# heli-sudoo/HKD-MPC

Hardware: AMD Instinct MI355X
Metric: batched DDP iters/sec (fwd+bwd), 4-phase 200-knot HKD fp64, batch=4096 (higher is better)
Workload: dtype f64

## Files before the change

### hkd-mpc_amd/csrc/hsddp_sweep.hip

```cpp
#include "hsddp_wave.h"

namespace hsddp {

using namespace hkd;

namespace sweep {

#ifndef HSDDP_STAMPS
#define HSDDP_STAMPS 0
#endif
#ifndef SWEEP_WPB2_WPE
#define SWEEP_WPB2_WPE 1
#endif
#if HSDDP_STAMPS
#define STAMP(n)                                                                              \
    do {                                                                                      \
        __builtin_amdgcn_sched_barrier(0);                                                    \
        unsigned long long t_;                                                                \
        asm volatile("s_waitcnt lgkmcnt(0)\n\ts_memtime %0\n\ts_waitcnt lgkmcnt(0)" : "=s"(t_)::"memory"); \
        __builtin_amdgcn_sched_barrier(0);                                                    \
        if (threadIdx.x == 0) {                                                               \
            if ((n) > 0) S.st[n] += t_ - S.tprev;                                             \
            S.tprev = t_;                                                                     \
        }                                                                                     \
    } while (0)
#else
#define STAMP(n) \
    do {         \
    } while (0)
#endif

#define SSYNC()                              \
    do {                                     \
        asm volatile("" ::: "memory");       \
        __builtin_amdgcn_sched_barrier(0);   \
    } while (0)

#define CSYNC()                                              \
    do {                                                     \
        asm volatile("s_waitcnt lgkmcnt(0)" ::: "memory");   \
        __builtin_amdgcn_s_barrier();                        \
        asm volatile("" ::: "memory");                       \
        __builtin_amdgcn_sched_barrier(0);                   \
    } while (0)

constexpr int HC = 12;
constexpr int MS = 26;
constexpr int TS = 14;
constexpr int WS = 25;
constexpr int V_SE = LQ_SE, V_D = 104, V_LX = 128, V_LU = 152, V_RB = 176, VW = 200;
static_assert(LQ_BW + 36 == V_D && LQ_LX + 24 == V_LX && LQ_LU + 24 == V_LU && LQ_RB + 24 == V_RB, "image layout");

template <typename real>
struct alignas(16) Lds {
    real img[2][VW];
    real zero[32];
    struct alignas(16) Item {
        real TI[24 * TS];
        real MI[25 * MS];
        real du[24];
        real pc[8];
    } it[2];
#if HSDDP_STAMPS
    unsigned long long st[12], tprev;
#endif
};
static_assert(sizeof(Lds<double>) <= 20480, "two waves per SIMD on 160 KB of LDS need <= 20 KB per wave");

template <typename real>
struct alignas(16) LdsCS {
    real img[2][2][VW];
    real zero[32];
    struct alignas(16) Item {
        real TI[24 * TS];
        real MZ[2][25 * MS];
        real du[24];
        real pc[8];
    } it[2];
    int fl[2];
};
static_assert(sizeof(LdsCS<double>) <= 40960, "four split workgroups per CU on 160 KB of LDS need <= 40 KB each");

template <typename real>
struct Pieces {
    static constexpr int E = 16 / sizeof(real);
    static constexpr int NA = V_D / E, ND = NX / E, NR = (LQW - V_D) / E, NP = NA + ND + NR;
    static constexpr int NI = (2 * NP + 63) / 64;
    static_assert(NP * E == VW && V_D % E == 0, "16-byte pieces");
};

template <typename real> struct Prec;
template <> struct Prec<double> {
    static DEV const double *lq(const Bufs &d) { return d.lq; }
    static DEV double *K(const Bufs &d) { return d.K; }
    static DEV const double *def(const Bufs &d, int b) { return kdbuf(work_buf(d, b)); }
    static constexpr int LQS = LQW;
};
template <> struct Prec<float> {
    static DEV const float *lq(const Bufs &d) { return d.lq32; }
    static DEV float *K(const Bufs &d) { return d.K32; }
    static DEV const float *def(const Bufs &d, int) { return d.def32; }
    static constexpr int LQS = LQW32;
};

template <typename real>
struct Item {
    int b;
    bool act;
    real reg;
    real *K;
    double *dU;
};

template <typename real>
struct Phase {
    int cmask;
    int xmask;
    real lxd;
    real xw;
    real dtr;
    real dtrz;
};


template <typename real, typename ItemT>
DEV void load_phase(const Params &p, const Bufs &d, ItemT &I, int b, int i, int pp, Phase<real> &ph)
{
    const int *cs = d.contacts + ((size_t)b * (p.P + 1) + i) * 4;
    int c[4];
#pragma unroll
    for (int l = 0; l < 4; ++l) c[l] = cs[l];
    ph.cmask = 0;
#pragma unroll
    for (int l = 0; l < 4; ++l) ph.cmask |= (c[l] != 0) << l;
    SSYNC();
    if (pp < 8) {
        const int cl = (ph.cmask >> (pp & 3)) & 1;
        I.pc[pp] = pp < 4 ? (cl ? (real)p.dt_m : (real)0) : (cl ? (real)0 : (real)p.dt);
    }
    SSYNC();
    const int pos = pp & 15, cq = (ph.cmask >> ((pos / 3) & 3)) & 1;
    ph.dtr = (real)(p.dt * (cq ? p.r_grf : p.r_qJd));
    const int cz = (ph.cmask >> ((pp < HC ? pp : 0) / 3)) & 1;
    ph.dtrz = (real)(p.dt * (cz ? p.r_qJd : p.r_grf));
    const int r = pp < NX ? pp : 0;
    double dg = p.dt * (r < 12 ? kparams()->qbase[r] : p.q_qJ * (1 - ((ph.cmask >> ((r - 12) / 3)) & 1)));
    ph.xmask = 0;
    ph.xw = 0;
    if (r >= 3 && r < 6) {
        const double fw = p.dt * (p.foot_gain * kparams()->foot_w[r - 3]);
#pragma unroll
        for (int l = 0; l < 4; ++l) dg += c[l] ? fw : 0.0;
        ph.xmask = ph.cmask;
        ph.xw = (real)fw;
    } else if (r >= 12) {
        const int m = r - 12;
        const double w = ((ph.cmask >> (m / 3)) & 1) ? p.dt * (p.foot_gain * kparams()->foot_w[m % 3]) : 0.0;
        dg += w;
        ph.xmask = 1;
        ph.xw = (real)w;
    }
    ph.lxd = (real)dg;
}

template <typename real>
DEV void fetch(Lds<real> &S, const real *rec0, const real *def0, const real *rec1, const real *def1, int lane)
{
    using PC = Pieces<real>;
    asm volatile("s_waitcnt lgkmcnt(0)" ::: "memory");
#pragma unroll
    for (int t = 0; t < PC::NI; ++t) {
        const int n = 64 * t + lane;
        if (n < 2 * PC::NP) {
            const int e = n >= PC::NP, q = n - e * PC::NP;
            const real *rec = e ? rec1 : rec0, *def = e ? def1 : def0;
            const real *src = q < PC::NA ? rec + PC::E * q : q < PC::NA + PC::ND ? def + PC::E * (q - PC::NA)
                                                                                 : rec + PC::E * (q - PC::ND);
            lds_dma16(src, (unsigned)(size_t)(&S.img[0][0]) + 1024u * t);
        }
    }
}

template <int W, typename real>
DEV void fetch_cs(LdsCS<real> &S, int q, const real *rec0, const real *def0, const real *rec1, const real *def1,
                  int lane)
{
    using PC = Pieces<real>;
    constexpr int H = (PC::NI + 1) / 2;
#pragma unroll
    for (int u = 0; u < H; ++u) {
        const int t = W * H + u;
        const int n = 64 * t + lane;
        if (t < PC::NI && n < 2 * PC::NP) {
            const int e = n >= PC::NP, qq = n - e * PC::NP;
            const real *rec = e ? rec1 : rec0, *def = e ? def1 : def0;
            const real *src = qq < PC::NA ? rec + PC::E * qq : qq < PC::NA + PC::ND ? def + PC::E * (qq - PC::NA)
                                                                                    : rec + PC::E * (qq - PC::ND);
            lds_dma16(src, (unsigned)(size_t)(&S.img[q][0][0]) + 1024u * t);
        }
    }
}

DEV constexpr int rb_index(int a, int b)
{
    return (a < b ? a : b) == 0 ? (a > b ? a : b) : (a < b ? a : b) == 1 ? 2 + (a > b ? a : b) : 5;
}

struct Lane {
    int lane, e, pp, pos;
    bool row;
    bool qlane;
    int rb[3];
    int xc0, xkind;
};

constexpr unsigned CS_COLS1 = (1u << 0) | (1u << 3) | (1u << 4) | (1u << 5) | (1u << 8) | (1u << 9) | (1u << 10) |
                              (1u << 11) | (1u << 18) | (1u << 19) | (1u << 21) | (1u << 22);
DEV constexpr int cs_wave(int c) { return (int)((CS_COLS1 >> c) & 1u); }
template <int W>
DEV constexpr bool cs_mine(int c) { return W < 0 || cs_wave(c) == W; }

template <int W = -1, typename real>
DEV void emit_SA(real (&acc)[NX], const real (&x)[NX], const real (&cf)[8], real dt)
{
    auto sw_row = [&](auto I) {
        constexpr int i = I;
        static_for<17>([&](auto Q) {
            if constexpr (cs_mine<W>(sw_col(Q))) vfma<sw_at(i, Q)>(acc[sw_col(Q)], cf, x[6 + i]);
        });
    };
    auto se_row = [&](auto I) {
        constexpr int i = I;
        static_for<5>([&](auto Q) {
            if constexpr (cs_mine<W>(se_col(Q))) vfma<V_SE + 5 * i + Q>(acc[se_col(Q)], cf, x[i]);
        });
    };
    sw_row(std::integral_constant<int, 0>{});
    se_row(std::integral_constant<int, 0>{});
    sw_row(std::integral_constant<int, 1>{});
    se_row(std::integral_constant<int, 1>{});
    sw_row(std::integral_constant<int, 2>{});
    se_row(std::integral_constant<int, 2>{});
    static_for<3>([&](auto A) {
        if constexpr (cs_mine<W>(9 + A)) acc[9 + A] = __builtin_fma(x[3 + A], dt, acc[9 + A]);
    });
}

template <int Q0 = 0, int Q1 = HC, typename real>
DEV void emit_Bc(real (&acc)[HC], real y6, real y7, real y8, const real *y9, const real *y12, const real (&bv)[4],
                 const real (&bq)[4], const real (&cf)[8])
{
#pragma unroll
    for (int q = Q0; q < Q1; ++q) acc[q] = __builtin_fma(y12[q], bq[q / 3], acc[q]);
#pragma unroll
    for (int q = Q0; q < Q1; ++q) acc[q] = __builtin_fma(y9[q % 3], bv[q / 3], acc[q]);
    static_for<Q1 - Q0>([&](auto Q) { vfma<bw_at(0, Q0 + Q)>(acc[Q0 + Q], cf, y6); });
    static_for<Q1 - Q0>([&](auto Q) { vfma<bw_at(1, Q0 + Q)>(acc[Q0 + Q], cf, y7); });
    static_for<Q1 - Q0>([&](auto Q) { vfma<bw_at(2, Q0 + Q)>(acc[Q0 + Q], cf, y8); });
}

template <typename real>
DEV void eliminate(real (&w)[HC], real (&w2)[HC], unsigned long long &bad)
{
    constexpr bool F64 = sizeof(real) == 8;
    constexpr int CH = F64 ? 13 : 9;
    real r, e, nf, nf2;
    {
        const real piv = row_bcast<0>(w[0]);
        bad |= __builtin_amdgcn_ballot_w64(!(piv > (real)1e-9));
        asm_rcp(r, piv);
        asm_nfma1(e, piv, r);
        asm_newton(r, e);
        if constexpr (F64) {
            asm_nfma1(e, piv, r);
            asm_newton(r, e);
        }
        asm_nmul(nf, w[0], r);
        asm_nmul(nf2, w2[0], r);
    }
    static_for<HC>([&](auto J) {
        constexpr int j = J, jn = j + 1;
        constexpr bool nx = jn < HC;
        real pivn = 0, rn = 0, en = 0, nfn = 0, nf2n = 0;
        if constexpr (nx) {
            bfma<j>(w2[jn], w[jn], nf2);
            fmac_row_bcast<j, false>(w[jn], nf);
        }
        constexpr int NO = nx ? HC - 2 - j : 0;
        constexpr int NT = (2 * NO > CH + 1) ? 2 * NO : CH + 1;
        static_for<NT>([&](auto T) {
            constexpr int t = T, i = jn + 1 + t / 2;
            if constexpr (t < 2 * NO) {
                if constexpr (t % 2 == 0)
                    bfma<j>(w2[i], w[i], nf2);
                else
                    fmac_row_bcast<j, false>(w[i], nf);
            }
            if constexpr (nx) {
                if constexpr (t == 1) pivn = row_bcast<(nx ? jn : 0)>(w[jn]);
                if constexpr (t == 3) asm_rcp(rn, pivn);
                if constexpr (t == 5) asm_nfma1(en, pivn, rn);
                if constexpr (t == 7) asm_newton(rn, en);
                if constexpr (F64 && t == 9) asm_nfma1(en, pivn, rn);
                if constexpr (F64 && t == 11) asm_newton(rn, en);
                if constexpr (t == CH) {
                    asm_nmul(nfn, w[jn], rn);
                    asm_nmul(nf2n, w2[jn], rn);
                }
            }
        });
        w[j] = nf;
        w2[j] = nf2;
        if constexpr (nx) {
            bad |= __builtin_amdgcn_ballot_w64(!(pivn > (real)1e-9));
            nf = nfn;
            nf2 = nf2n;
        }
    });
    static_for<HC - 1>([&](auto Jr) {
        constexpr int j = HC - 1 - Jr;
        static_for<j>([&](auto Ii) {
            constexpr int i = j - 1 - Ii;
            bfma<j>(w2[i], w[i], w2[j]);
        });
    });
}

template <int W, bool DV, typename real, typename LdsT>
DEV void knot(const Params &p, LdsT &S, const Lane &L, const Phase<real> &ph, const Item<real> &it, int kc,
              real (&h)[NX], real &g, bool &live, bool first, bool more, int ib, int par, const real *nrec0,
              const real *ndef0, const real *nrec1, const real *ndef1, double &dvs)
{
    constexpr bool CS = W >= 0;
    constexpr int Q0 = CS ? 6 * W : 0, Q1 = CS ? Q0 + 6 : HC;
    auto &I = S.it[L.e];
    const real *img;
    real *ma = nullptr, *za = nullptr;
    if constexpr (CS) {
        img = S.img[ib][L.e];
        ma = I.MZ[par];
        za = I.MZ[par ^ 1];
    } else {
        img = S.img[L.e];
    }
    auto MA = [&]() -> real * { if constexpr (CS) return ma; else return I.MI; };
    auto ZA = [&]() -> real * { if constexpr (CS) return za; else return I.MI; };
    const int pp = L.pp, pos = L.pos;
    const real dt = (real)p.dt;
    const real reg = it.reg;
    if constexpr (!CS) STAMP(0);
    if (first) {
        asm volatile("s_waitcnt vmcnt(0)" ::: "memory");
        if constexpr (CS) CSYNC();
    }
    real cf[8];
#pragma unroll
    for (int k = 0; k < 8; ++k) cf[k] = img[16 * k + pos];
    real bv[4], bq[4];
#pragma unroll
    for (int l = 0; l < 4; ++l) { bv[l] = I.pc[l]; bq[l] = I.pc[4 + l]; }
    if constexpr (!CS) STAMP(1);
    real t[HC], ga[4] = {g, 0, 0, 0};
#pragma unroll
    for (int q = 0; q < HC; ++q) t[q] = 0;
    emit_Bc<Q0, Q1>(t, h[6], h[7], h[8], h + 9, h + 12, bv, bq, cf);
    static_for<NX>([&](auto C) { vfma<V_D + C>(ga[C & 3], cf, h[C]); });
    const real gn = (ga[0] + ga[1]) + (ga[2] + ga[3]);
    pin(t);
    real h9[NX];
#pragma unroll
    for (int j = 0; j < 9; ++j) h9[j] = h[j];
#pragma unroll
    for (int j = 9; j < NX; ++j) h9[j] = 0;
    SSYNC();
    real (&m)[NX] = h;
    emit_SA<W>(m, h9, cf, dt);
    pin(t);
    pin(m);
    if (L.row) {
        static_for<NX>([&](auto C) {
            if constexpr (cs_mine<W>(C)) MA()[pp * MS + C] = m[C];
        });
        if constexpr (W <= 0) MA()[pp * MS + NX] = gn;
#pragma unroll
        for (int q = Q0; q < Q1; ++q) I.TI[pp * TS + q] = t[q];
    }
    if constexpr (CS) CSYNC(); else SSYNC();
    if constexpr (!CS) STAMP(2);
    const int pc = pp < MS - 1 ? pp : MS - 1;
    real mc[NX];
#pragma unroll
    for (int j = 0; j < NX; ++j) mc[j] = MA()[j * MS + pc];
    real w2[HC];
#pragma unroll
    for (int l = 0; l < 4; ++l) {
        const real *lcp = pp == NX ? img + V_LU + (((ph.cmask >> l) & 1) ? 3 * l : 12 + 3 * l) : S.zero;
#pragma unroll
        for (int a = 0; a < 3; ++a) w2[3 * l + a] = lcp[a];
    }
    emit_SA<W>(m, mc, cf, dt);
    emit_Bc(w2, mc[6], mc[7], mc[8], mc + 9, mc + 12, bv, bq, cf);
    pin(m);
    pin(w2);
    if constexpr (!CS) STAMP(3);
    if (pp <= NX) {
#pragma unroll
        for (int c = 0; c < NX; ++c)
            if (cs_mine<W>(c)) ZA()[pp * MS + c] = m[c];
        if constexpr (W <= 0) {
            ZA()[pp * MS + NX] = 0;
            ZA()[pp * MS + NX + 1] = 0;
        }
    }
    SSYNC();
    if (L.row) {
        real *zr = ZA() + pp * MS;
        if (cs_mine<W>(pp)) lds_add(zr + pp, ph.lxd + reg);
#pragma unroll
        for (int t2 = 0; t2 < 4; ++t2) {
            const int xc = L.xkind == 1 ? L.xc0 + 3 * t2 : L.xc0;
            if (((ph.xmask >> t2) & 1) && cs_mine<W>(xc)) lds_add(zr + xc, -ph.xw);
        }
    }
    if constexpr (CS) CSYNC(); else SSYNC();
    const real *zrow = L.row ? ZA() + pp * MS : S.zero;
    real qxx[NX], zc[NX];
    if constexpr (CS) {
        static_for<NX>([&](auto C) {
            if constexpr (cs_mine<W>(C)) {
                qxx[C] = zrow[C];
                zc[C] = ZA()[C * MS + pc];
            }
        });
        static_for<NX>([&](auto C) {
            if constexpr (cs_mine<W>(C)) qxx[C] = __builtin_fma(zc[C], (real)0.5, qxx[C] * (real)0.5);
        });
    } else {
#pragma unroll
        for (int c = 0; c < NX; ++c) qxx[c] = zrow[c];
#pragma unroll
        for (int c = 0; c < NX; ++c) zc[c] = ZA()[c * MS + pc];
        pin(qxx);
        pin(zc);
#pragma unroll
        for (int c = 0; c < NX; ++c) qxx[c] *= (real)0.5;
#pragma unroll
        for (int c = 0; c < NX; ++c) qxx[c] = __builtin_fma(zc[c], (real)0.5, qxx[c]);
        pin(qxx);
    }
    const real qx = img[V_LX + (L.row ? pp : 0)] + (gn + ZA()[NX * MS + pc]);
    if constexpr (!CS) STAMP(4);
    real tcol[18];
#pragma unroll
    for (int j = 0; j < 18; ++j) tcol[j] = I.TI[(6 + j) * TS + pos];
    real lbr[3];
    const int aq = pos % 3;
#pragma unroll
    for (int a = 0; a < 3; ++a) lbr[a] = (L.qlane ? img + L.rb[a] : S.zero + a)[0] + (a == aq ? ph.dtr + reg : (real)0);
    const int lq = pos / 3;
    real w[HC];
#pragma unroll
    for (int q = 0; q < HC; ++q) w[q] = (L.qlane && lq == q / 3) ? lbr[q % 3] : (real)0;
    emit_Bc(w, tcol[0], tcol[1], tcol[2], tcol + 3, tcol + 6, bv, bq, cf);
    pin(w);
    const bool zl = pp < HC;
    const int du_z = ((ph.cmask >> ((zl ? pp : 0) / 3)) & 1) ? 12 + pp : pp;
    const real quz = img[zl ? V_LU + du_z : V_LU];
    const real qzz = ph.dtrz + reg;
    if (more) {
        if constexpr (CS) fetch_cs<W>(S, ib ^ 1, nrec0, ndef0, nrec1, ndef1, L.lane);
        else fetch(S, nrec0, ndef0, nrec1, ndef1, L.lane);
    }
    if constexpr (!CS) STAMP(5);
    real quxs[HC];
#pragma unroll
    for (int q = 0; q < HC; ++q) quxs[q] = (L.row || (DV && pp == NX)) ? w2[q] : (real)0;
    pin(quxs);
    unsigned long long bad = __builtin_amdgcn_ballot_w64(zl && !(qzz > (real)1e-9));
    eliminate(w, w2, bad);
    const bool okh = L.e ? (bad >> 32) == 0 : (bad & 0xffffffffull) == 0;
    live = live && okh;
    const bool st = live;
    if constexpr (!CS) STAMP(6);
    if (pp == NX)
#pragma unroll
        for (int q = 0; q < HC; ++q) I.du[(((ph.cmask >> (q / 3)) & 1) ? 0 : 12) + q] = w2[q];
    if (zl) I.du[du_z] = -(quz / qzz);
    SSYNC();
    real ka[HC], kb[HC];
#pragma unroll
    for (int q = 0; q < HC; ++q) row_pair_last(w2[q], ka[q], kb[q]);
    real gq4[4] = {qx, 0, 0, 0};
    static_for<HC>([&](auto Q) { bfma<8>(gq4[Q & 3], kb[Q], quxs[Q]); });
    const real gq = (gq4[0] + gq4[1]) + (gq4[2] + gq4[3]);
    if constexpr (DV) {
        real dq = 0;
        static_for<HC>([&](auto Q) { bfma<8>(dq, kb[Q], quxs[Q]); });
        const double v = pp == NX ? (double)dq : zl ? (double)quz * (double)(-(quz / qzz)) : 0.0;
        if (st) dvs += v;
    }
    if constexpr (!CS) STAMP(7);
    if constexpr (CS) {
        static_for<NX>([&](auto C) {
            if constexpr (cs_mine<W>(C)) h[C] = qxx[C];
        });
    } else {
#pragma unroll
        for (int c = 0; c < NX; ++c) h[c] = qxx[c];
    }
    static_for<HC>([&](auto Q) {
        static_for<NX>([&](auto C) {
            constexpr int c = C;
            if constexpr (cs_mine<W>(c)) {
                if constexpr (c < 16)
                    bfma<c & 15>(h[c], ka[Q], quxs[Q]);
                else
                    bfma<c & 15>(h[c], kb[Q], quxs[Q]);
            }
        });
    });
    if constexpr (DV)
        if (!L.row)
            static_for<NX>([&](auto C) {
                if constexpr (cs_mine<W>(C)) h[C] = 0;
            });
    if constexpr (!CS) STAMP(8);
    g = L.row ? gq : (real)0;
    if constexpr (CS)
        if (L.row)
            static_for<NX>([&](auto C) {
                if constexpr (cs_mine<W>(C)) MA()[pp * MS + C] = h[C];
            });
    asm volatile("s_waitcnt vmcnt(0)" ::: "memory");
    if (st) {
        real *Kg = it.K + (size_t)kc * KCW;
        if constexpr (W <= 0) {
#pragma unroll
            for (int q = 0; q < HC; ++q) Kg[q * NX + pos] = ka[q];
        }
        if constexpr (W != 0) {
            if (pos < NX - 16)
#pragma unroll
                for (int q = 0; q < HC; ++q) Kg[q * NX + 16 + pos] = kb[q];
            if (L.row) it.dU[(size_t)kc * NX + pp] = I.du[pp];
        }
    }
    if constexpr (CS) {
        CSYNC();
        static_for<NX>([&](auto C) {
            if constexpr (!cs_mine<W>(C)) h[C] = L.row ? MA()[pp * MS + C] : (real)0;
        });
    }
    SSYNC();
    if constexpr (!CS) STAMP(9);
}

template <typename real, bool EL, bool DV, int CSW = -1, typename LdsT = Lds<real>>
DEV int sweep_pair(const Params &p, const Bufs &d, LdsT &S, const Lane &L, const Item<real> &it, double &dv)
{
    constexpr bool CS = CSW >= 0;
    int ib = 0, par = 0;
    double dvs = 0.0;
    const int pp = L.pp;
    const real *lqg = Prec<real>::lq(d);
    const int b = it.b;
    const int b0 = __builtin_amdgcn_readlane(b, 0), b1 = __builtin_amdgcn_readlane(b, 32);
    const real *defg0 = Prec<real>::def(d, b0), *defg1 = Prec<real>::def(d, b1);
    bool live = it.act;
    int fail = -1;
    real h[NX], g = 0;
    const auto PL = layout_of<EL>(d, b0);
    const int P = PL.P();
    for (int i = P - 1; i >= 0; --i) {
        Phase<real> ph;
        load_phase<real>(p, d, S.it[L.e], b, i, pp, ph);
        const double *rec = d.term + ((size_t)b * p.P + i) * TW;
        if (i == P - 1) {
#pragma unroll
            for (int c = 0; c < NX; ++c) h[c] = L.row ? (real)rec[TM_PHIXX + pp * NX + c] : (real)0;
            g = L.row ? (real)rec[TM_PHIX + pp] : (real)0;
        } else {
            auto &I = S.it[L.e];
            real *WI;
            if constexpr (CS) {
                WI = I.MZ[0];
                CSYNC();
            } else {
                WI = I.MI;
            }
            const double *Px = rec + TM_PX;
            real wr[NX];
#pragma unroll
            for (int c = 0; c < NX; ++c) wr[c] = 0;
            static_for<3>([&](auto Kc) {
                real px[12];
#pragma unroll
                for (int k = 0; k < 12; ++k) px[k] = (real)Px[192 * Kc + 16 * k + L.pos];
                if constexpr (sizeof(real) == 4) dpp_ready(px);
                static_for<8>([&](auto Kk) {
                    static_for<NX>([&](auto Cc) { vfma<NX * Kk + Cc>(wr[Cc], px, h[8 * Kc + Kk]); });
                });
            });
            SSYNC();
            if (L.row) {
#pragma unroll
                for (int c = 0; c < NX; ++c) WI[pp * WS + c] = wr[c];
                WI[pp * WS + NX] = g;
            }
            SSYNC();
            const int pc = pp < NX ? pp : NX;
            real wc[NX];
#pragma unroll
            for (int j = 0; j < NX; ++j) wc[j] = WI[j * WS + pc];
            real vr[NX];
#pragma unroll
            for (int c = 0; c < NX; ++c) vr[c] = 0;
            static_for<3>([&](auto Kc) {
                real px[12];
#pragma unroll
                for (int k = 0; k < 12; ++k) px[k] = (real)Px[192 * Kc + 16 * k + L.pos];
                if constexpr (sizeof(real) == 4) dpp_ready(px);
                static_for<8>([&](auto Jj) {
                    static_for<NX>([&](auto Cc) { vfma<NX * Jj + Cc>(vr[Cc], px, wc[8 * Kc + Jj]); });
                });
            });
            SSYNC();
            if (pp == NX)
#pragma unroll
                for (int c = 0; c < NX; ++c) WI[NX * WS + c] = vr[c];
            SSYNC();
            const real gp = WI[NX * WS + (L.row ? pp : 0)];
#pragma unroll
            for (int c = 0; c < NX; ++c) h[c] = L.row ? (real)rec[TM_PHIXX + pp * NX + c] + vr[c] : (real)0;
            g = L.row ? (real)rec[TM_PHIX + pp] + gp : (real)0;
            SSYNC();
            if constexpr (CS) CSYNC();
        }
        const int N = PL.N(i), s0 = PL.s0(i), k0 = PL.k0(i);
        auto recp = [&](int bb, int k) { return lqg + ((size_t)bb * p.Kc + k0 + k) * Prec<real>::LQS; };
        auto defp0 = [&](int k) { return defg0 + ((size_t)b0 * p.S + s0 + k + 1) * NX; };
        auto defp1 = [&](int k) { return defg1 + ((size_t)b1 * p.S + s0 + k + 1) * NX; };
        if constexpr (CS) fetch_cs<CSW>(S, ib, recp(b0, N - 1), defp0(N - 1), recp(b1, N - 1), defp1(N - 1), L.lane);
        else fetch(S, recp(b0, N - 1), defp0(N - 1), recp(b1, N - 1), defp1(N - 1), L.lane);
        int k = N - 1;
#pragma unroll 1
        for (; k >= 0; --k) {
            const bool more = k > 0;
            const int kn = more ? k - 1 : 0;
            const bool was = live;
            knot<CSW, DV>(p, S, L, ph, it, k0 + k, h, g, live, k == N - 1, more, ib, par, recp(b0, kn), defp0(kn),
                          recp(b1, kn), defp1(kn), dvs);
            if constexpr (CS) {
                ib ^= more ? 1 : 0;
                par ^= 1;
            }
            if (was && !live) fail = k0 + k;
            if (!__builtin_amdgcn_ballot_w64(live)) break;
        }
        asm volatile("s_waitcnt vmcnt(0)" ::: "memory");
        if (!__builtin_amdgcn_ballot_w64(live)) break;
        const real *d0 = (L.e ? defg1 : defg0) + ((size_t)b * p.S + s0) * NX;
        real dc[2] = {d0[L.pos], L.pos < NX - 16 ? d0[16 + L.pos] : (real)0};
        real a = 0;
        static_for<NX>([&](auto Cc) { vfma<Cc>(a, dc, h[Cc]); });
        if (L.row) g += a;
        if (p.store_value && live && L.row && CSW <= 0) {
            double *V = d.value0 + ((size_t)b * p.P + i) * (NX + NN);
#pragma unroll
            for (int c = 0; c < NX; ++c) V[NX + pp * NX + c] = (double)h[c];
            V[pp] = (double)g;
        }
    }
    if constexpr (DV) {
#pragma unroll
        for (int o = 16; o > 0; o >>= 1) dvs += __shfl_xor(dvs, o);
    }
    dv = dvs;
    return it.act ? fail : -1;
}

constexpr int STAGE_SLOTS = 512;

template <typename ItemT>
DEV double *cost_stage(const Params &p, ItemT &item)
{
    const bool fits = p.S <= STAGE_SLOTS && 2 * (size_t)p.S * sizeof(double) <= sizeof(ItemT);
    return fits ? reinterpret_cast<double *>(&item) : nullptr;
}

template <bool EL>
DEV void element_cost(const Params &p, const Bufs &d, int b, int lane, double *stg, double &cost, double &feas)
{
    const auto LY = layout_of<EL>(d, b);
    const int P = LY.P(), g = lane & 31;
    const double *c = d.slot_cost + (size_t)b * p.S, *f = d.slot_feas + (size_t)b * p.S;
    if (stg) {
        const int Sel = LY.S();
#pragma unroll
        for (int t = 0; t < STAGE_SLOTS / 32; ++t) {
            const int sl = g + 32 * t;
            if (sl < Sel) {
                stg[sl] = c[sl];
                stg[p.S + sl] = f[sl];
            }
        }
        __builtin_amdgcn_fence(__ATOMIC_RELEASE, "wavefront");
        __builtin_amdgcn_wave_barrier();
        __builtin_amdgcn_fence(__ATOMIC_ACQUIRE, "wavefront");
        c = stg;
        f = stg + p.S;
    }
    double ci = 0.0, fi = 0.0;
    if (g < P) {
        const int N = LY.N(g), s0 = LY.s0(g);
#pragma unroll 10
        for (int k = 0; k < N; ++k) {
            ci += c[s0 + k];
            fi += f[s0 + k];
        }
        ci += c[s0 + N];
        fi += f[s0 + N];
    }
    cost = 0.0; feas = 0.0;
    for (int i = 0; i < P; ++i) {
        cost += __shfl(ci, (lane & 32) + i);
        feas += __shfl(fi, (lane & 32) + i);
    }
    feas = sqrt(feas);
}

DEV Lane make_lane()
{
    Lane L;
    L.lane = threadIdx.x & 63;
    L.e = L.lane >> 5;
    L.pp = L.lane & 31;
    L.pos = L.lane & 15;
    L.row = L.pp < NX;
    L.qlane = L.pos < HC;
    const int lq = (L.qlane ? L.pos : 0) / 3, aq = L.pos % 3;
#pragma unroll
    for (int a = 0; a < 3; ++a) L.rb[a] = V_RB + 6 * lq + rb_index(aq, a);
    L.xkind = (L.pp >= 3 && L.pp < 6) ? 1 : (L.pp >= 12 && L.pp < NX) ? 2 : 0;
    L.xc0 = L.xkind == 1 ? 12 + (L.pp - 3) : L.xkind == 2 ? 3 + (L.pp - 12) % 3 : MS - 1;
    return L;
}

template <typename LdsT>
DEV void zero_init(LdsT &S, int lane)
{
    if (lane < 32) S.zero[lane] = 0;
    SSYNC();
}

template <bool EL, typename Idx>
DEV void pair_element(const Params &p, const Bufs &d, const Lane &L, Idx pair, int &bv, bool &valid)
{
    int b;
    if constexpr (EL) {
        const int e0 = d.pairs[2 * pair], e1 = d.pairs[2 * pair + 1];
        b = L.e ? e1 : e0;
        valid = b >= 0;
        bv = valid ? b : (L.e ? e0 : e1);
    } else {
        b = 2 * pair + L.e;
        valid = b < p.B;
        bv = valid ? b : p.B - 1;
    }
}

}

using namespace sweep;

template <typename real, bool EL, bool DV, int WPB>
__global__ __launch_bounds__(64 * WPB) __attribute__((amdgpu_waves_per_eu(WPB == 2 ? SWEEP_WPB2_WPE : 2))) void k_riccati(Params p, Bufs d)
{
    __shared__ Lds<real> SS[WPB];
    const int wv = WPB > 1 ? __builtin_amdgcn_readfirstlane((int)(threadIdx.x >> 6)) : 0;
    Lds<real> &S = SS[wv];
    const int pair = (int)blockIdx.x * WPB + wv;
    const Lane L = make_lane();
    zero_init(S, L.lane);
#if HSDDP_STAMPS
    if (L.lane < 12) S.st[L.lane] = 0;
#endif
    if constexpr (EL)
        if (pair >= p.n_pairs) return;
    int bv;
    bool valid;
    pair_element<EL>(p, d, L, pair, bv, valid);
    ElemState &E = d.el[bv];
    bool act = valid && !E.done && !E.inner_done;
    if (!__builtin_amdgcn_ballot_w64(act)) return;
    double ecost, efeas;
    {
        double *stg = cost_stage(p, S.it[L.e]);
        element_cost<EL>(p, d, bv, L.lane, stg, ecost, efeas);
        SSYNC();
    }
    double reg = E.reg;
    Item<real> it;
    it.b = bv;
    it.K = Prec<real>::K(d) + (size_t)bv * p.Kc * KCW;
    it.dU = d.dU + (size_t)bv * p.Kc * NX;
    bool need = act, ok = false;
    double dvk = 0.0;
    for (int attempt = 0; __builtin_amdgcn_ballot_w64(need); ++attempt) {
        it.act = need;
        it.reg = (real)reg;
        double dv;
        const int fk = sweep_pair<real, EL, DV>(p, d, S, L, it, dv);
        if (need) {
            if (fk < 0) {
                ok = true;
                need = false;
                dvk = dv;
            } else {
                bool deferred = false;
                if (attempt == 0 && p.retry_cap > 0) {
                    int f = 0;
                    if (L.pp == 0) {
                        f = atomicAdd(d.retry_count, 1);
                        if (f < p.retry_cap) d.retry_list[f] = RetryEntry{bv, 0, reg};
                    }
                    f = __shfl(f, L.lane & 32);
                    deferred = f < p.retry_cap;
                }
                if (deferred) {
                    need = false;
                    if (L.pp == 0) { E.iters += 1; E.cost = ecost; E.feas = efeas; E.accepted = 0; }
                    act = false;
                } else {
                    reg = fmax(reg * p.update_regularization, 1e-03);
                    if (reg > 1e2 || attempt >= MAX_REG_ATTEMPTS) need = false;
                }
            }
        }
    }
#if HSDDP_STAMPS
    SSYNC();
    if (L.lane < 12) d.dbg[(size_t)__builtin_amdgcn_readfirstlane(bv) * 16 + L.lane] += S.st[L.lane];
#endif
    if (act && L.pp == 0) {
        double rn = reg / 20;
        if (rn < 1e-06) rn = 0;
        E.iters += 1; E.cost = ecost; E.feas = efeas; E.accepted = 0;
        if (ok) E.reg = rn;
        else { E.reg = rn; E.status = 1; E.done = 1; E.ls_active = 0; }
        if (DV && ok) merit_step(p, E, dvk, -dvk);
    }
}

template <bool EL, bool DV, int W>
DEV void riccati_cs_wave(const Params &p, const Bufs &d, LdsCS<double> &S)
{
    using real = double;
    const Lane L = make_lane();
    int bv;
    bool valid;
    pair_element<EL>(p, d, L, blockIdx.x, bv, valid);
    ElemState &E = d.el[bv];
    bool act = valid && !E.done && !E.inner_done;
    if (!__builtin_amdgcn_ballot_w64(act)) return;
    double ecost = 0, efeas = 0;
    if (W == 0) {
        double *stg = cost_stage(p, S.it[L.e]);
        element_cost<EL>(p, d, bv, L.lane, stg, ecost, efeas);
    }
    CSYNC();
    double reg = E.reg;
    Item<real> it;
    it.b = bv;
    it.K = d.K + (size_t)bv * p.Kc * KCW;
    it.dU = d.dU + (size_t)bv * p.Kc * NX;
    bool need = act, ok = false;
    double dvk = 0.0;
    for (int attempt = 0; __builtin_amdgcn_ballot_w64(need); ++attempt) {
        it.act = need;
        it.reg = (real)reg;
        double dv;
        const int fk = sweep_pair<real, EL, DV, W>(p, d, S, L, it, dv);
        if (attempt == 0 && p.retry_cap > 0) {
            if (W == 0 && need && fk >= 0 && L.pp == 0) {
                const int f = atomicAdd(d.retry_count, 1);
                if (f < p.retry_cap) d.retry_list[f] = RetryEntry{bv, 0, reg};
                S.fl[L.e] = f;
            }
            CSYNC();
        }
        if (need) {
            if (fk < 0) {
                ok = true;
                need = false;
                dvk = dv;
            } else {
                const bool deferred = attempt == 0 && p.retry_cap > 0 && S.fl[L.e] < p.retry_cap;
                if (deferred) {
                    need = false;
                    if (W == 0 && L.pp == 0) { E.iters += 1; E.cost = ecost; E.feas = efeas; E.accepted = 0; }
                    act = false;
                } else {
                    reg = fmax(reg * p.update_regularization, 1e-03);
                    if (reg > 1e2 || attempt >= MAX_REG_ATTEMPTS) need = false;
                }
            }
        }
        CSYNC();
    }
    if (W == 0 && act && L.pp == 0) {
        double rn = reg / 20;
        if (rn < 1e-06) rn = 0;
        E.iters += 1; E.cost = ecost; E.feas = efeas; E.accepted = 0;
        E.reg = rn;
        if (!ok) { E.status = 1; E.done = 1; E.ls_active = 0; }
        if (DV && ok) merit_step(p, E, dvk, -dvk);
    }
}

template <bool EL, bool DV>
__global__ __launch_bounds__(128) __attribute__((amdgpu_waves_per_eu(2))) void k_riccati_cs(Params p, Bufs d)
{
    __shared__ LdsCS<double> S;
    zero_init(S, threadIdx.x & 63);
    __syncthreads();
    if (threadIdx.x < 64) riccati_cs_wave<EL, DV, 0>(p, d, S);
    else riccati_cs_wave<EL, DV, 1>(p, d, S);
}

template <typename real, bool EL, bool DV>
__global__ __launch_bounds__(64, 2) void k_riccati_retry(Params p, Bufs d)
{
    __shared__ Lds<real> S;
    const Lane L = make_lane();
    zero_init(S, L.lane);
    const int n = min(*d.retry_count, p.retry_cap);
    const int mpad = p.retry_m + (p.retry_m & 1);
    const int item = 2 * blockIdx.x + L.e, f = item / mpad, a = item % mpad + 1;
    bool act = f < n && a <= p.retry_m;
    if (!__builtin_amdgcn_ballot_w64(act)) return;
    const int fv = f < n ? f : 0;
    const RetryEntry e = d.retry_list[fv];
    double reg = e.reg;
    for (int t = 0; t < a; ++t) reg = fmax(reg * p.update_regularization, 1e-03);
    const int av = a <= p.retry_m ? a : p.retry_m;
    int *flag = d.retry_flag + fv * p.retry_m + (av - 1);
    if (act && reg > 1e2) {
        if (L.pp == 0) *flag = 2;
        act = false;
    }
    if (!__builtin_amdgcn_ballot_w64(act)) return;
    const size_t slot = (size_t)fv * p.retry_m + (av - 1);
    Item<real> it;
    it.b = e.b;
    it.act = act;
    it.reg = (real)reg;
    it.K = (real *)d.retry_K + slot * p.Kc * KCW;
    it.dU = d.retry_dU + slot * p.Kc * NX;
    double dv;
    const int fk = sweep_pair<real, EL, DV>(p, d, S, L, it, dv);
    if (act && L.pp == 0) *flag = fk < 0 ? 1 : -1 - fk;
    if (DV && act && L.pp == 0) d.retry_dv[slot] = dv;
}

template <typename real>
__global__ __launch_bounds__(64) void k_riccati_select(Params p, Bufs d)
{
    const int f = blockIdx.x, lane = threadIdx.x;
    if (f >= min(*d.retry_count, p.retry_cap)) return;
    const RetryEntry e = d.retry_list[f];
    const size_t b = e.b;
    double reg = e.reg;
    int win = 0;
    for (int a = 1; a <= p.retry_m; ++a) {
        reg = fmax(reg * p.update_regularization, 1e-03);
        if (reg > 1e2) break;
        if (d.retry_flag[f * p.retry_m + a - 1] == 1) { win = a; break; }
    }
    real *Ko = Prec<real>::K(d) + b * p.Kc * KCW;
    double *dUo = d.dU + b * p.Kc * NX;
    if (win) {
        const size_t slot = (size_t)f * p.retry_m + (win - 1);
        const real *Ks = (const real *)d.retry_K + slot * p.Kc * KCW;
        const double *Us = d.retry_dU + slot * p.Kc * NX;
        for (size_t q = lane; q < (size_t)p.Kc * KCW; q += 64) Ko[q] = Ks[q];
        for (size_t q = lane; q < (size_t)p.Kc * NX; q += 64) dUo[q] = Us[q];
    } else {
        const int *fl = d.retry_flag + f * p.retry_m;
        auto source = [&](int kc) {
            int src = 0;
            for (int a = 1; a <= p.retry_m && fl[a - 1] != 2; ++a)
                if (-1 - fl[a - 1] < kc) src = a;
            return src;
        };
        const real *K0 = (const real *)d.retry_K + (size_t)f * p.retry_m * p.Kc * KCW;
        const double *U0 = d.retry_dU + (size_t)f * p.retry_m * p.Kc * NX;
        for (size_t q = lane; q < (size_t)p.Kc * KCW; q += 64) {
            const int a = source((int)(q / KCW));
            if (a) Ko[q] = K0[(size_t)(a - 1) * p.Kc * KCW + q];
        }
        for (size_t q = lane; q < (size_t)p.Kc * NX; q += 64) {
            const int a = source((int)(q / NX));
            if (a) dUo[q] = U0[(size_t)(a - 1) * p.Kc * NX + q];
        }
    }
    if (lane == 0) {
        ElemState &E = d.el[b];
        double rn = reg / 20;
        if (rn < 1e-06) rn = 0;
        E.reg = rn;
        if (!win) { E.status = 1; E.done = 1; E.ls_active = 0; }
        else if (p.ms0) {
            const double dv = d.retry_dv[(size_t)f * p.retry_m + (win - 1)];
            merit_step(p, E, dv, -dv);
        }
    }
}

static int device_cus()
{
    static int cus[64] = {0};
    int dev = 0;
    hipGetDevice(&dev);
    if (dev < 0 || dev >= 64) return 256;
    if (!cus[dev]) {
        int n = 0;
        if (hipDeviceGetAttribute(&n, hipDeviceAttributeMultiprocessorCount, dev) != hipSuccess || n < 1) n = 256;
        cus[dev] = n;
    }
    return cus[dev];
}

static bool sweep_split(const Params &p)
{
    if (p.fp32) return false;
    const char *e = std::getenv("HSDDP_SWEEP_SPLIT");
    if (e && *e) return *e != '0';
    return (p.elem_layout ? p.n_pairs : (p.B + 1) / 2) <= device_cus();
}

static int sweep_wpb(const Params &p)
{
    if (p.fp32) return 1;
    const char *e = std::getenv("HSDDP_SWEEP_WPB");
    if (e && *e) return *e == '2' ? 2 : 1;
    const int pairs = p.elem_layout ? p.n_pairs : (p.B + 1) / 2, cus = device_cus();
    return pairs > cus && pairs <= 4 * cus ? 2 : 1;
}

void launch_riccati(const Params &p, const Bufs &d, hipStream_t st)
{
    const dim3 g1((unsigned)(p.elem_layout ? p.n_pairs : (p.B + 1) / 2));
#define HSDDP_RIC(kern, grid, real)                                                                          \
    do {                                                                                                     \
        if (p.ms0) {                                                                                         \
            if (p.elem_layout) hipLaunchKernelGGL((kern<real, true, true>), grid, dim3(64), 0, st, p, d);      \
            else hipLaunchKernelGGL((kern<real, false, true>), grid, dim3(64), 0, st, p, d);                   \
        } else {                                                                                             \
            if (p.elem_layout) hipLaunchKernelGGL((kern<real, true, false>), grid, dim3(64), 0, st, p, d);     \
            else hipLaunchKernelGGL((kern<real, false, false>), grid, dim3(64), 0, st, p, d);                  \
        }                                                                                                    \
    } while (0)
    const int wpb = sweep_wpb(p);
    const dim3 gw((unsigned)(((p.elem_layout ? p.n_pairs : (p.B + 1) / 2) + wpb - 1) / wpb));
#define HSDDP_RIC_W(real, W)                                                                                   \
    do {                                                                                                       \
        if (p.ms0) {                                                                                           \
            if (p.elem_layout) hipLaunchKernelGGL((k_riccati<real, true, true, W>), gw, dim3(64 * W), 0, st, p, d);  \
            else hipLaunchKernelGGL((k_riccati<real, false, true, W>), gw, dim3(64 * W), 0, st, p, d);               \
        } else {                                                                                               \
            if (p.elem_layout) hipLaunchKernelGGL((k_riccati<real, true, false, W>), gw, dim3(64 * W), 0, st, p, d); \
            else hipLaunchKernelGGL((k_riccati<real, false, false, W>), gw, dim3(64 * W), 0, st, p, d);              \
        }                                                                                                      \
    } while (0)
    if (p.fp32) HSDDP_RIC_W(float, 1);
    else if (sweep_split(p)) {
        if (p.ms0) {
            if (p.elem_layout) hipLaunchKernelGGL((k_riccati_cs<true, true>), g1, dim3(128), 0, st, p, d);
            else hipLaunchKernelGGL((k_riccati_cs<false, true>), g1, dim3(128), 0, st, p, d);
        } else {
            if (p.elem_layout) hipLaunchKernelGGL((k_riccati_cs<true, false>), g1, dim3(128), 0, st, p, d);
            else hipLaunchKernelGGL((k_riccati_cs<false, false>), g1, dim3(128), 0, st, p, d);
        }
    } else if (wpb == 2) HSDDP_RIC_W(double, 2);
    else HSDDP_RIC_W(double, 1);
#undef HSDDP_RIC_W
    if (p.retry_cap > 0) {
        const dim3 gr((unsigned)(p.retry_cap * (p.retry_m + (p.retry_m & 1)) / 2)), gs((unsigned)p.retry_cap);
        if (p.fp32) {
            HSDDP_RIC(k_riccati_retry, gr, float);
            hipLaunchKernelGGL(k_riccati_select<float>, gs, dim3(64), 0, st, p, d);
        } else {
            HSDDP_RIC(k_riccati_retry, gr, double);
            hipLaunchKernelGGL(k_riccati_select<double>, gs, dim3(64), 0, st, p, d);
        }
    }
#undef HSDDP_RIC
}

}
```

Before: 1.112 million.

## Specialize Riccati knot loop on compile-time contact masks for trot phases

Pulls the per-phase backward knot loop out into a noinline function templated on the contact mask. For the two trot gait masks it drops, at compile time, the FMAs that belong to swing-leg or stance-leg columns in the B and S·A products. The phase state is spilled through LDS and a struct around the call, and global pointers are tagged with an address-space attribute. The specialized path only runs when both paired elements share the same mask and every lane is live; otherwise a generic noinline version runs. That adds call overhead and LDS round-trips per phase, and may change register allocation.

```diff
diff --git a/hkd-mpc_amd/csrc/hsddp_sweep.hip b/hkd-mpc_amd/csrc/hsddp_sweep.hip
--- a/hkd-mpc_amd/csrc/hsddp_sweep.hip
+++ b/hkd-mpc_amd/csrc/hsddp_sweep.hip
@@ -103,13 +103,16 @@
     static constexpr int LQS = LQW32;
 };
 
+template <typename T>
+using Global = __attribute__((address_space(1))) T *;
+
 template <typename real>
 struct Item {
     int b;
     bool act;
     real reg;
-    real *K;
-    double *dU;
+    Global<real> K;
+    Global<double> dU;
 };
 
 template <typename real>
@@ -213,6 +216,7 @@
     int rb[3];
     int xc0, xkind;
 };
+DEV Lane make_lane();
 
 constexpr unsigned CS_COLS1 = (1u << 0) | (1u << 3) | (1u << 4) | (1u << 5) | (1u << 8) | (1u << 9) | (1u << 10) |
                               (1u << 11) | (1u << 18) | (1u << 19) | (1u << 21) | (1u << 22);
@@ -220,13 +224,20 @@
 template <int W>
 DEV constexpr bool cs_mine(int c) { return W < 0 || cs_wave(c) == W; }
 
-template <int W = -1, typename real>
+template <int MASK>
+DEV constexpr bool stance(int l) { return MASK < 0 || ((MASK >> l) & 1); }
+template <int MASK>
+DEV constexpr bool swing(int l) { return MASK < 0 || !((MASK >> l) & 1); }
+template <int MASK>
+DEV constexpr bool sw_live(int q) { return q < 9 || stance<MASK>((q - 9) >> 1); }
+
+template <int W = -1, int MASK = -1, typename real>
 DEV void emit_SA(real (&acc)[NX], const real (&x)[NX], const real (&cf)[8], real dt)
 {
     auto sw_row = [&](auto I) {
         constexpr int i = I;
         static_for<17>([&](auto Q) {
-            if constexpr (cs_mine<W>(sw_col(Q))) vfma<sw_at(i, Q)>(acc[sw_col(Q)], cf, x[6 + i]);
+            if constexpr (cs_mine<W>(sw_col(Q)) && sw_live<MASK>(Q)) vfma<sw_at(i, Q)>(acc[sw_col(Q)], cf, x[6 + i]);
         });
     };
     auto se_row = [&](auto I) {
@@ -246,17 +257,25 @@
     });
 }
 
-template <int Q0 = 0, int Q1 = HC, typename real>
+template <int Q0 = 0, int Q1 = HC, int MASK = -1, typename real>
 DEV void emit_Bc(real (&acc)[HC], real y6, real y7, real y8, const real *y9, const real *y12, const real (&bv)[4],
                  const real (&bq)[4], const real (&cf)[8])
 {
 #pragma unroll
-    for (int q = Q0; q < Q1; ++q) acc[q] = __builtin_fma(y12[q], bq[q / 3], acc[q]);
-#pragma unroll
-    for (int q = Q0; q < Q1; ++q) acc[q] = __builtin_fma(y9[q % 3], bv[q / 3], acc[q]);
-    static_for<Q1 - Q0>([&](auto Q) { vfma<bw_at(0, Q0 + Q)>(acc[Q0 + Q], cf, y6); });
-    static_for<Q1 - Q0>([&](auto Q) { vfma<bw_at(1, Q0 + Q)>(acc[Q0 + Q], cf, y7); });
-    static_for<Q1 - Q0>([&](auto Q) { vfma<bw_at(2, Q0 + Q)>(acc[Q0 + Q], cf, y8); });
+    for (int q = Q0; q < Q1; ++q)
+        if (swing<MASK>(q / 3)) acc[q] = __builtin_fma(y12[q], bq[q / 3], acc[q]);
+#pragma unroll
+    for (int q = Q0; q < Q1; ++q)
+        if (stance<MASK>(q / 3)) acc[q] = __builtin_fma(y9[q % 3], bv[q / 3], acc[q]);
+    static_for<Q1 - Q0>([&](auto Q) {
+        if constexpr (stance<MASK>((Q0 + Q) / 3)) vfma<bw_at(0, Q0 + Q)>(acc[Q0 + Q], cf, y6);
+    });
+    static_for<Q1 - Q0>([&](auto Q) {
+        if constexpr (stance<MASK>((Q0 + Q) / 3)) vfma<bw_at(1, Q0 + Q)>(acc[Q0 + Q], cf, y7);
+    });
+    static_for<Q1 - Q0>([&](auto Q) {
+        if constexpr (stance<MASK>((Q0 + Q) / 3)) vfma<bw_at(2, Q0 + Q)>(acc[Q0 + Q], cf, y8);
+    });
 }
 
 template <typename real>
@@ -326,8 +345,8 @@
     });
 }
 
-template <int W, bool DV, typename real, typename LdsT>
-DEV void knot(const Params &p, LdsT &S, const Lane &L, const Phase<real> &ph, const Item<real> &it, int kc,
+template <int W, bool DV, int MASK = -1, typename real, typename LdsT>
+DEV void knot(real dt, LdsT &S, const Lane &L, const Phase<real> &ph, const Item<real> &it, int kc,
               real (&h)[NX], real &g, bool &live, bool first, bool more, int ib, int par, const real *nrec0,
               const real *ndef0, const real *nrec1, const real *ndef1, double &dvs)
 {
@@ -346,8 +365,8 @@
     auto MA = [&]() -> real * { if constexpr (CS) return ma; else return I.MI; };
     auto ZA = [&]() -> real * { if constexpr (CS) return za; else return I.MI; };
     const int pp = L.pp, pos = L.pos;
-    const real dt = (real)p.dt;
     const real reg = it.reg;
+    const int cmask = MASK >= 0 ? MASK : ph.cmask;
     if constexpr (!CS) STAMP(0);
     if (first) {
         asm volatile("s_waitcnt vmcnt(0)" ::: "memory");
@@ -363,7 +382,7 @@
     real t[HC], ga[4] = {g, 0, 0, 0};
 #pragma unroll
     for (int q = 0; q < HC; ++q) t[q] = 0;
-    emit_Bc<Q0, Q1>(t, h[6], h[7], h[8], h + 9, h + 12, bv, bq, cf);
+    emit_Bc<Q0, Q1, MASK>(t, h[6], h[7], h[8], h + 9, h + 12, bv, bq, cf);
     static_for<NX>([&](auto C) { vfma<V_D + C>(ga[C & 3], cf, h[C]); });
     const real gn = (ga[0] + ga[1]) + (ga[2] + ga[3]);
     pin(t);
@@ -374,7 +393,7 @@
     for (int j = 9; j < NX; ++j) h9[j] = 0;
     SSYNC();
     real (&m)[NX] = h;
-    emit_SA<W>(m, h9, cf, dt);
+    emit_SA<W, MASK>(m, h9, cf, dt);
     pin(t);
     pin(m);
     if (L.row) {
@@ -394,12 +413,12 @@
     real w2[HC];
 #pragma unroll
     for (int l = 0; l < 4; ++l) {
-        const real *lcp = pp == NX ? img + V_LU + (((ph.cmask >> l) & 1) ? 3 * l : 12 + 3 * l) : S.zero;
+        const real *lcp = pp == NX ? img + V_LU + (((cmask >> l) & 1) ? 3 * l : 12 + 3 * l) : S.zero;
 #pragma unroll
         for (int a = 0; a < 3; ++a) w2[3 * l + a] = lcp[a];
     }
-    emit_SA<W>(m, mc, cf, dt);
-    emit_Bc(w2, mc[6], mc[7], mc[8], mc + 9, mc + 12, bv, bq, cf);
+    emit_SA<W, MASK>(m, mc, cf, dt);
+    emit_Bc<0, HC, MASK>(w2, mc[6], mc[7], mc[8], mc + 9, mc + 12, bv, bq, cf);
     pin(m);
     pin(w2);
     if constexpr (!CS) STAMP(3);
@@ -423,7 +442,7 @@
         }
     }
     if constexpr (CS) CSYNC(); else SSYNC();
-    const real *zrow = L.row ? ZA() + pp * MS : S.zero;
+    const real *zrow = (const real *)__builtin_assume_aligned(L.row ? ZA() + pp * MS : S.zero, 16);
     real qxx[NX], zc[NX];
     if constexpr (CS) {
         static_for<NX>([&](auto C) {
@@ -461,10 +480,10 @@
     real w[HC];
 #pragma unroll
     for (int q = 0; q < HC; ++q) w[q] = (L.qlane && lq == q / 3) ? lbr[q % 3] : (real)0;
-    emit_Bc(w, tcol[0], tcol[1], tcol[2], tcol + 3, tcol + 6, bv, bq, cf);
+    emit_Bc<0, HC, MASK>(w, tcol[0], tcol[1], tcol[2], tcol + 3, tcol + 6, bv, bq, cf);
     pin(w);
     const bool zl = pp < HC;
-    const int du_z = ((ph.cmask >> ((zl ? pp : 0) / 3)) & 1) ? 12 + pp : pp;
+    const int du_z = ((cmask >> ((zl ? pp : 0) / 3)) & 1) ? 12 + pp : pp;
     const real quz = img[zl ? V_LU + du_z : V_LU];
     const real qzz = ph.dtrz + reg;
     if (more) {
@@ -484,7 +503,7 @@
     if constexpr (!CS) STAMP(6);
     if (pp == NX)
 #pragma unroll
-        for (int q = 0; q < HC; ++q) I.du[(((ph.cmask >> (q / 3)) & 1) ? 0 : 12) + q] = w2[q];
+        for (int q = 0; q < HC; ++q) I.du[(((cmask >> (q / 3)) & 1) ? 0 : 12) + q] = w2[q];
     if (zl) I.du[du_z] = -(quz / qzz);
     SSYNC();
     real ka[HC], kb[HC];
@@ -533,7 +552,7 @@
             });
     asm volatile("s_waitcnt vmcnt(0)" ::: "memory");
     if (st) {
-        real *Kg = it.K + (size_t)kc * KCW;
+        const Global<real> Kg = it.K + (size_t)kc * KCW;
         if constexpr (W <= 0) {
 #pragma unroll
             for (int q = 0; q < HC; ++q) Kg[q * NX + pos] = ka[q];
@@ -555,8 +574,87 @@
     if constexpr (!CS) STAMP(9);
 }
 
-template <typename real, bool EL, bool DV, int CSW = -1, typename LdsT = Lds<real>>
-DEV int sweep_pair(const Params &p, const Bufs &d, LdsT &S, const Lane &L, const Item<real> &it, double &dv)
+template <int MASK, int CSW, bool DV, typename real, typename LdsT>
+DEV void phase_knots(real dt, LdsT &S, const Lane &L, const Phase<real> &ph, const Item<real> &it, int N, int kc0,
+                     const real *rec0, const real *def0, const real *rec1, const real *def1, real (&h)[NX], real &g,
+                     bool &live, int &fail, double &dvs, int &ib, int &par)
+{
+    constexpr bool CS = CSW >= 0;
+    constexpr int LQS = Prec<real>::LQS;
+    if constexpr (CS) fetch_cs<CSW>(S, ib, rec0 + (size_t)(N - 1) * LQS, def0 + (size_t)(N - 1) * NX, rec1 + (size_t)(N - 1) * LQS,
+                                    def1 + (size_t)(N - 1) * NX, L.lane);
+    else fetch(S, rec0 + (size_t)(N - 1) * LQS, def0 + (size_t)(N - 1) * NX, rec1 + (size_t)(N - 1) * LQS,
+               def1 + (size_t)(N - 1) * NX, L.lane);
+    int k = N - 1;
+#pragma unroll 1
+    for (; k >= 0; --k) {
+        const bool more = k > 0;
+        const int kn = more ? k - 1 : 0;
+        const bool was = live;
+        knot<CSW, DV, MASK>(dt, S, L, ph, it, kc0 + k, h, g, live, k == N - 1, more, ib, par, rec0 + (size_t)kn * LQS,
+                            def0 + (size_t)kn * NX, rec1 + (size_t)kn * LQS, def1 + (size_t)kn * NX, dvs);
+        if constexpr (CS) {
+            ib ^= more ? 1 : 0;
+            par ^= 1;
+        }
+        if (was && !live) fail = kc0 + k;
+        if (!__builtin_amdgcn_ballot_w64(live)) break;
+    }
+}
+
+constexpr int MASK_TROT_A = (1 << 0) | (1 << 3), MASK_TROT_B = (1 << 1) | (1 << 2);
+
+struct PhaseOut {
+    double dvs;
+    int live, fail;
+};
+
+template <typename T>
+DEV T *uniform_ptr(T *q)
+{
+    const size_t v = (size_t)q;
+    const unsigned lo = __builtin_amdgcn_readfirstlane((unsigned)v), hi = __builtin_amdgcn_readfirstlane((unsigned)(v >> 32));
+    return (T *)(((size_t)hi << 32) | lo);
+}
+
+template <int MASK, bool DV, int WPE, typename real>
+__device__ __attribute__((noinline)) void phase_knots_masked(unsigned lds, int flags, real lxd, real xw, real dtr,
+                                                             real dtrz, real reg, Global<real> K, Global<double> dU,
+                                                             real dt, int N, int k0, const real *rec0, const real *def0,
+                                                             const real *rec1, const real *def1, PhaseOut *io)
+{
+    typedef __attribute__((address_space(3))) Lds<real> *LdsPtr;
+    static_assert(alignof(Lds<real>) == 16, "the masked address bits");
+    Lds<real> &S = *(Lds<real> *)(LdsPtr)(size_t)(__builtin_amdgcn_readfirstlane(lds) & ~15u);
+    const Lane L = make_lane();
+    Phase<real> ph;
+    ph.cmask = MASK >= 0 ? MASK : (flags & 15);
+    ph.xmask = (flags >> 4) & 15; ph.lxd = lxd; ph.xw = xw; ph.dtr = dtr; ph.dtrz = dtrz;
+    Item<real> it;
+    it.b = 0; it.act = true; it.reg = reg; it.K = K; it.dU = dU;
+    real *row = S.it[L.e].MI + L.pp * MS;
+    real h[NX], g = L.row ? row[NX] : (real)0;
+#pragma unroll
+    for (int j = 0; j < NX; ++j) h[j] = L.row ? row[j] : (real)0;
+    SSYNC();
+    double dvs = io->dvs;
+    bool live = io->live != 0;
+    int fail = io->fail, ib = 0, par = 0;
+    phase_knots<MASK, -1, DV>(uniform(dt), S, L, ph, it, __builtin_amdgcn_readfirstlane(N), __builtin_amdgcn_readfirstlane(k0),
+                              uniform_ptr(rec0), uniform_ptr(def0), uniform_ptr(rec1), uniform_ptr(def1), h, g, live, fail,
+                              dvs, ib, par);
+    if (L.row) {
+#pragma unroll
+        for (int j = 0; j < NX; ++j) row[j] = h[j];
+        row[NX] = g;
+    }
+    SSYNC();
+    io->dvs = dvs; io->live = live; io->fail = fail;
+}
+
+template <typename real, bool EL, bool DV, int CSW = -1, int WPE = 2, typename LdsT = Lds<real>>
+DEV int sweep_pair(const Params &p, const Bufs &d, LdsT &S, const Lane &L, const Item<real> &it, double &dv,
+                   bool masks = false)
 {
     constexpr bool CS = CSW >= 0;
     int ib = 0, par = 0;
@@ -637,25 +735,34 @@
             if constexpr (CS) CSYNC();
         }
         const int N = PL.N(i), s0 = PL.s0(i), k0 = PL.k0(i);
-        auto recp = [&](int bb, int k) { return lqg + ((size_t)bb * p.Kc + k0 + k) * Prec<real>::LQS; };
-        auto defp0 = [&](int k) { return defg0 + ((size_t)b0 * p.S + s0 + k + 1) * NX; };
-        auto defp1 = [&](int k) { return defg1 + ((size_t)b1 * p.S + s0 + k + 1) * NX; };
-        if constexpr (CS) fetch_cs<CSW>(S, ib, recp(b0, N - 1), defp0(N - 1), recp(b1, N - 1), defp1(N - 1), L.lane);
-        else fetch(S, recp(b0, N - 1), defp0(N - 1), recp(b1, N - 1), defp1(N - 1), L.lane);
-        int k = N - 1;
-#pragma unroll 1
-        for (; k >= 0; --k) {
-            const bool more = k > 0;
-            const int kn = more ? k - 1 : 0;
-            const bool was = live;
-            knot<CSW, DV>(p, S, L, ph, it, k0 + k, h, g, live, k == N - 1, more, ib, par, recp(b0, kn), defp0(kn),
-                          recp(b1, kn), defp1(kn), dvs);
-            if constexpr (CS) {
-                ib ^= more ? 1 : 0;
-                par ^= 1;
+        const real *rec0 = lqg + ((size_t)b0 * p.Kc + k0) * Prec<real>::LQS, *def0 = defg0 + ((size_t)b0 * p.S + s0 + 1) * NX;
+        const real *rec1 = lqg + ((size_t)b1 * p.Kc + k0) * Prec<real>::LQS, *def1 = defg1 + ((size_t)b1 * p.S + s0 + 1) * NX;
+        if constexpr (CS || DV) {
+            phase_knots<-1, CSW, DV>((real)p.dt, S, L, ph, it, N, k0, rec0, def0, rec1, def1, h, g, live, fail, dvs, ib, par);
+        } else {
+            real *row = S.it[L.e].MI + pp * MS;
+            if (L.row) {
+#pragma unroll
+                for (int c = 0; c < NX; ++c) row[c] = h[c];
+                row[NX] = g;
             }
-            if (was && !live) fail = k0 + k;
-            if (!__builtin_amdgcn_ballot_w64(live)) break;
+            SSYNC();
+            const int m0 = __builtin_amdgcn_readlane(ph.cmask, 0), m1 = __builtin_amdgcn_readlane(ph.cmask, 32);
+            const bool both = masks && m0 == m1 && __builtin_amdgcn_ballot_w64(live) == ~0ull;
+            const int flags = ph.cmask | (ph.xmask << 4);
+            PhaseOut o{dvs, live, fail};
+#define HSDDP_PHASE(MASK)                                                                                              \
+    phase_knots_masked<MASK, DV, WPE, real>((unsigned)(size_t)&S, flags, ph.lxd, ph.xw, ph.dtr, ph.dtrz, it.reg, it.K, \
+                                            it.dU, (real)p.dt, N, k0, rec0, def0, rec1, def1, &o)
+            if (both && m0 == MASK_TROT_A) HSDDP_PHASE(MASK_TROT_A);
+            else if (both && m0 == MASK_TROT_B) HSDDP_PHASE(MASK_TROT_B);
+            else HSDDP_PHASE(-1);
+#undef HSDDP_PHASE
+            dvs = o.dvs; live = o.live != 0; fail = o.fail;
+#pragma unroll
+            for (int c = 0; c < NX; ++c) h[c] = L.row ? row[c] : (real)0;
+            g = L.row ? row[NX] : (real)0;
+            SSYNC();
         }
         asm volatile("s_waitcnt vmcnt(0)" ::: "memory");
         if (!__builtin_amdgcn_ballot_w64(live)) break;
@@ -774,7 +881,7 @@
 using namespace sweep;
 
 template <typename real, bool EL, bool DV, int WPB>
-__global__ __launch_bounds__(64 * WPB) __attribute__((amdgpu_waves_per_eu(WPB == 2 ? SWEEP_WPB2_WPE : 2))) void k_riccati(Params p, Bufs d)
+__global__ __launch_bounds__(64 * WPB) __attribute__((amdgpu_waves_per_eu(WPB == 2 ? SWEEP_WPB2_WPE : 2))) void k_riccati(Params p, Bufs d, int masks)
 {
     __shared__ Lds<real> SS[WPB];
     const int wv = WPB > 1 ? __builtin_amdgcn_readfirstlane((int)(threadIdx.x >> 6)) : 0;
@@ -802,15 +909,15 @@
     double reg = E.reg;
     Item<real> it;
     it.b = bv;
-    it.K = Prec<real>::K(d) + (size_t)bv * p.Kc * KCW;
-    it.dU = d.dU + (size_t)bv * p.Kc * NX;
+    it.K = (Global<real>)(Prec<real>::K(d) + (size_t)bv * p.Kc * KCW);
+    it.dU = (Global<double>)(d.dU + (size_t)bv * p.Kc * NX);
     bool need = act, ok = false;
     double dvk = 0.0;
     for (int attempt = 0; __builtin_amdgcn_ballot_w64(need); ++attempt) {
         it.act = need;
         it.reg = (real)reg;
         double dv;
-        const int fk = sweep_pair<real, EL, DV>(p, d, S, L, it, dv);
+        const int fk = sweep_pair<real, EL, DV, -1, (WPB == 2 ? SWEEP_WPB2_WPE : 2)>(p, d, S, L, it, dv, masks != 0);
         if (need) {
             if (fk < 0) {
                 ok = true;
@@ -872,8 +979,8 @@
     double reg = E.reg;
     Item<real> it;
     it.b = bv;
-    it.K = d.K + (size_t)bv * p.Kc * KCW;
-    it.dU = d.dU + (size_t)bv * p.Kc * NX;
+    it.K = (Global<real>)(d.K + (size_t)bv * p.Kc * KCW);
+    it.dU = (Global<double>)(d.dU + (size_t)bv * p.Kc * NX);
     bool need = act, ok = false;
     double dvk = 0.0;
     for (int attempt = 0; __builtin_amdgcn_ballot_w64(need); ++attempt) {
@@ -929,7 +1036,7 @@
 }
 
 template <typename real, bool EL, bool DV>
-__global__ __launch_bounds__(64, 2) void k_riccati_retry(Params p, Bufs d)
+__global__ __launch_bounds__(64, 2) void k_riccati_retry(Params p, Bufs d, int masks)
 {
     __shared__ Lds<real> S;
     const Lane L = make_lane();
@@ -955,10 +1062,10 @@
     it.b = e.b;
     it.act = act;
     it.reg = (real)reg;
-    it.K = (real *)d.retry_K + slot * p.Kc * KCW;
-    it.dU = d.retry_dU + slot * p.Kc * NX;
+    it.K = (Global<real>)((real *)d.retry_K + slot * p.Kc * KCW);
+    it.dU = (Global<double>)(d.retry_dU + slot * p.Kc * NX);
     double dv;
-    const int fk = sweep_pair<real, EL, DV>(p, d, S, L, it, dv);
+    const int fk = sweep_pair<real, EL, DV>(p, d, S, L, it, dv, masks != 0);
     if (act && L.pp == 0) *flag = fk < 0 ? 1 : -1 - fk;
     if (DV && act && L.pp == 0) d.retry_dv[slot] = dv;
 }
@@ -1039,6 +1146,12 @@
     return (p.elem_layout ? p.n_pairs : (p.B + 1) / 2) <= device_cus();
 }
 
+static int sweep_masks()
+{
+    const char *e = std::getenv("HSDDP_SWEEP_MASKS");
+    return e && *e == '0' ? 0 : 1;
+}
+
 static int sweep_wpb(const Params &p)
 {
     if (p.fp32) return 1;
@@ -1054,23 +1167,23 @@
 #define HSDDP_RIC(kern, grid, real)                                                                          \
     do {                                                                                                     \
         if (p.ms0) {                                                                                         \
-            if (p.elem_layout) hipLaunchKernelGGL((kern<real, true, true>), grid, dim3(64), 0, st, p, d);      \
-            else hipLaunchKernelGGL((kern<real, false, true>), grid, dim3(64), 0, st, p, d);                   \
+            if (p.elem_layout) hipLaunchKernelGGL((kern<real, true, true>), grid, dim3(64), 0, st, p, d, masks); \
+            else hipLaunchKernelGGL((kern<real, false, true>), grid, dim3(64), 0, st, p, d, masks);            \
         } else {                                                                                             \
-            if (p.elem_layout) hipLaunchKernelGGL((kern<real, true, false>), grid, dim3(64), 0, st, p, d);     \
-            else hipLaunchKernelGGL((kern<real, false, false>), grid, dim3(64), 0, st, p, d);                  \
+            if (p.elem_layout) hipLaunchKernelGGL((kern<real, true, false>), grid, dim3(64), 0, st, p, d, masks); \
+            else hipLaunchKernelGGL((kern<real, false, false>), grid, dim3(64), 0, st, p, d, masks);           \
         }                                                                                                    \
     } while (0)
-    const int wpb = sweep_wpb(p);
+    const int wpb = sweep_wpb(p), masks = sweep_masks();
     const dim3 gw((unsigned)(((p.elem_layout ? p.n_pairs : (p.B + 1) / 2) + wpb - 1) / wpb));
 #define HSDDP_RIC_W(real, W)                                                                                   \
     do {                                                                                                       \
         if (p.ms0) {                                                                                           \
-            if (p.elem_layout) hipLaunchKernelGGL((k_riccati<real, true, true, W>), gw, dim3(64 * W), 0, st, p, d);  \
-            else hipLaunchKernelGGL((k_riccati<real, false, true, W>), gw, dim3(64 * W), 0, st, p, d);               \
+            if (p.elem_layout) hipLaunchKernelGGL((k_riccati<real, true, true, W>), gw, dim3(64 * W), 0, st, p, d, masks);  \
+            else hipLaunchKernelGGL((k_riccati<real, false, true, W>), gw, dim3(64 * W), 0, st, p, d, masks);        \
         } else {                                                                                               \
-            if (p.elem_layout) hipLaunchKernelGGL((k_riccati<real, true, false, W>), gw, dim3(64 * W), 0, st, p, d); \
-            else hipLaunchKernelGGL((k_riccati<real, false, false, W>), gw, dim3(64 * W), 0, st, p, d);              \
+            if (p.elem_layout) hipLaunchKernelGGL((k_riccati<real, true, false, W>), gw, dim3(64 * W), 0, st, p, d, masks); \
+            else hipLaunchKernelGGL((k_riccati<real, false, false, W>), gw, dim3(64 * W), 0, st, p, d, masks);       \
         }                                                                                                      \
     } while (0)
     if (p.fp32) HSDDP_RIC_W(float, 1);
```

After: 1.138 million (median of 6 runs). 2.4% higher.
